# loryruta/gl-radix-sort

Measured on AMD Instinct MI355X. Metric: Mkeys/s sorting 2^28 uint32 key+val; % HBM roofline; 1/2/4/8 GPU, higher is better.
Workload: dtype u32; 1 GPU; 2^28 uint32 key + uint32 val pairs, uniform-random full-range keys, vals=iota, in-place stable radix sort, 1x MI355X; pairs_per_gpu=268435456, key_distribution=uniform, parallelism=single, device=AMD Radeon Graphics (gfx950:sramecc+:xnack-), 256 CUs, 288.0 GiB, device 0

## Files before the change

gl-radix-sort_amd/csrc/glu_sort_object.hpp:

```cpp
#pragma once
#include <algorithm>
#include <chrono>
#include <cmath>
#include <cstdlib>
#include <cstring>
#include <mutex>
#include <string>
#include <vector>

#include "glu_batch_host.hpp"
#include "radix_sort_kernels.hpp"

namespace glu_hip
{
namespace host
{
constexpr int kMaxRadix = 256;
constexpr int kMaxBlocksPerCu = 4;

template<int THREADS_, int KPT_, int BLOCKS_PER_CU_, bool CARRY_>
struct Geometry
{
    static constexpr int THREADS = THREADS_, KPT = KPT_, BLOCKS_PER_CU = BLOCKS_PER_CU_, TILE = THREADS_ * KPT_;
    static constexpr bool CARRY = CARRY_;
};
template<typename KeyT, int BITS, bool LARGE>
struct PairGeometry;
template<> struct PairGeometry<uint32_t, 8, true> : Geometry<1024, 12, 1, true> {};
template<> struct PairGeometry<uint32_t, 4, true> : Geometry<1024, 12, 1, true> {};
#ifndef GLU_SMALL_THREADS
#define GLU_SMALL_THREADS 512
#define GLU_SMALL_KPT 8
#define GLU_SMALL_BLOCKS_PER_CU 3
#endif
template<> struct PairGeometry<uint32_t, 8, false> : Geometry<GLU_SMALL_THREADS, GLU_SMALL_KPT, GLU_SMALL_BLOCKS_PER_CU, false> {};
template<> struct PairGeometry<uint32_t, 4, false> : Geometry<GLU_SMALL_THREADS, GLU_SMALL_KPT, GLU_SMALL_BLOCKS_PER_CU, false> {};
template<> struct PairGeometry<uint64_t, 8, true> : Geometry<512, 16, 1, true> {};
template<> struct PairGeometry<uint64_t, 4, true> : Geometry<1024, 8, 1, true> {};
template<> struct PairGeometry<uint64_t, 8, false> : Geometry<256, 8, 4, false> {};
template<> struct PairGeometry<uint64_t, 4, false> : Geometry<256, 8, 4, false> {};
template<typename KeyT, int BITS, bool LARGE, bool VALS = true>
struct GeometryFor : PairGeometry<KeyT, BITS, LARGE> {};
template<> struct GeometryFor<uint32_t, 8, true, false> : Geometry<1024, 20, 1, true> {};

#ifndef GLU_LINES_KPT_U32
#define GLU_LINES_KPT_U32 10
#endif
#ifndef GLU_LINES_KPT_U64
#define GLU_LINES_KPT_U64 6
#endif
template<typename KeyT, int BITS, bool VALS>
struct LinesGeometry : Geometry<1024, GLU_LINES_KPT_U32, 1, true> {};
#ifndef GLU_LINES_KPT_SEG
#define GLU_LINES_KPT_SEG 10
#endif
struct SegLinesGeometry : Geometry<1024, GLU_LINES_KPT_SEG, 1, true> {};
template<> struct LinesGeometry<uint32_t, 8, false> : Geometry<1024, 16, 1, true> {};
template<> struct LinesGeometry<uint32_t, 4, true> : Geometry<1024, 12, 1, true> {};
template<> struct LinesGeometry<uint32_t, 4, false> : Geometry<1024, 16, 1, true> {};
template<> struct LinesGeometry<uint64_t, 8, true> : Geometry<1024, GLU_LINES_KPT_U64, 1, true> {};
template<> struct LinesGeometry<uint64_t, 8, false> : Geometry<1024, 10, 1, true> {};
#ifndef GLU_LINES_KPT_U64_4BIT
#define GLU_LINES_KPT_U64_4BIT 8
#endif
template<> struct LinesGeometry<uint64_t, 4, true> : Geometry<1024, GLU_LINES_KPT_U64_4BIT, 1, true> {};
template<> struct LinesGeometry<uint64_t, 4, false> : Geometry<1024, 10, 1, true> {};
}
}

using namespace glu_hip;
using namespace glu_hip::host;

struct glu_radix_sort_s
{
    Scratch keys;
    Scratch vals;
    Scratch table;
    Scratch plan;
    Scratch pair_t2;
    Scratch pair_table;
    Scratch pair_ranges;
    Scratch pair_sub;
    Scratch pair_wide;
    Scratch seg_desc;
    Scratch seg_zero;
    bool last_planned = false;
    Scratch batch_lists;
    LastBatch last_batch;
    struct SegStage
    {
        void* host = nullptr;
        size_t size = 0;
        hipEvent_t copied = nullptr;
        bool in_flight = false;
    };
    SegStage seg_stage[16];
    uint32_t seg_stage_next = 0;
    Scratch long_image, long_hdr;
    Scratch long_bits;
    Scratch seg_gate;
    bool seg_finish = true;
    bool last_seg_finish_attempted = false;
    uint32_t last_seg_finish_capacity = 0, last_seg_finish_runs = 0, last_seg_finish_tile = 0, last_seg_finish_split = 0;
    uint32_t seg_split_max = 0;
    uint32_t seg_split_min = 0;
    uint32_t finish_rank_bits = 16;
    uint32_t seg_split_geo = 3;
    uint32_t seg_max_geo = 4;
    uint32_t digit_bits = 8;
    uint32_t max_blocks = 0;
    uint32_t reserved_cus = 0;
    bool force_small = false;
    bool no_single_block = false;
    bool no_fused_scan = false;
    bool no_plan = false;
    bool tune_scratch = true;
    bool tuning = false;
    uint32_t tuned_spacer_mib = 0, tuned_candidates = 0; double tuned_ms = 0, tuned_worst_ms = 0;
    bool no_lines = false;
    bool nt_stores = true;
    size_t nt_min_bytes = (size_t) 320 << 20;
    bool no_bit_shortcut = false;
    bool equal_shares = false;
    bool pairs = true;
    uint32_t last_pair_roles[kPlanMaxPasses] = {};
    size_t pair_min = 0;
    uint32_t pair_unit_div = 16;
    hipEvent_t after_histogram_event = nullptr;
    Scratch finish_lengths;
    Scratch finish_starts;
    Scratch finish_crowded;
    hipStream_t side = nullptr;
    hipEvent_t ev_fork = nullptr, ev_unit = nullptr, ev_fork2 = nullptr, ev_join = nullptr;
    bool fork_behind = true;
    bool ensure_side()
    {
        if (side) return true;
        if (hipStreamCreateWithFlags(&side, hipStreamNonBlocking) != hipSuccess) return side = nullptr, false;
        for (hipEvent_t* e : {&ev_fork, &ev_unit, &ev_fork2, &ev_join})
            if (hipEventCreateWithFlags(e, hipEventDisableTiming) != hipSuccess) return false;
        return true;
    }
    bool lds_finish = true;
    bool long_runs = true;
    size_t finish_min = 0;
    uint32_t* finish_hint = nullptr;
    uint32_t finish_seq = 0, finish_seq_acted_on = 0, finish_wait = 0;
    uint32_t finish_last_geo = 0;
    bool finish_last_refused = false;
    bool device_top = true;
    uint32_t top_floor = 0;
    bool last_device_top = false;
    uint32_t finish_top = 0;
    uint32_t last_finish_top = 0;
    uint32_t finish_backoff = 0;
    bool last_finish_attempted = false;
    bool last_finish_long_ok = false;
    uint32_t last_finish_capacity = 0;
    size_t large_min = 0;
    int profiling = 0;
    std::vector<hipEvent_t> events;
    size_t events_used = 0;
    std::vector<hipEvent_t> slots;
    hipEvent_t next_event()
    {
        if (events_used == events.size())
        {
            hipEvent_t e;
            if (hipEventCreate(&e) != hipSuccess) return nullptr;
            events.push_back(e);
        }
        return events[events_used++];
    }
    std::vector<uint8_t> pass_kinds;
    std::vector<uint32_t> pass_seqs;
    uint32_t cur_seq = 0;
    Scratch finish_outcomes;
    uint8_t cur_kind = 0;
    bool cur_behind = false;
    void mark(hipStream_t stream, bool around_data_kernel = false)
    {
        if (!profiling) return;
        if (slots.size() % 4 == 0) pass_kinds.push_back(cur_kind), pass_seqs.push_back(cur_seq);
        hipEvent_t e = nullptr;
        if (profiling == 1 || (around_data_kernel && !cur_behind))
            if ((e = next_event()) != nullptr) (void) hipEventRecord(e, stream);
        slots.push_back(e);
    }
};

namespace glu_hip
{
namespace host
{
constexpr size_t kPairMinKeyBytes = (size_t) 1 << 28;
constexpr size_t finish_min_count(size_t key_size) { return key_size == 8 ? (size_t) 3 << 21 : (size_t) 7 << 22; }
constexpr size_t kPlanMinCount = (size_t) 1 << 22;

inline uint32_t usable_cus(const glu_radix_sort_s* s)
{
    return (uint32_t) std::max<int>(1, g_dev.num_cus - (int) s->reserved_cus);
}

struct PlanArgs
{
    PassPlan* plan = nullptr;
    uint32_t pass = 0;
    bool may_skip = false;
    int pair_role = 0;
    uint32_t shift2 = 0, bits2 = 0;
    uint32_t flags = 0;
    bool behind_attempt = false;
    uint32_t finish_geo_first = 0, finish_geo_last = 0;
    uint32_t finish_first_ordinary = 0, finish_num_ordinary = 0;
    uint32_t finish_seq = 0, finish_top_bit = 0, finish_key_bits = 0;
    bool finish_long_ok = false;
    bool fork_side = false;
    bool unitsum_side = false;
};

constexpr size_t kSmallResidentPerCU = 4;

template<typename KeyT, int BITS>
size_t large_tiles_from(const glu_radix_sort_s* s, bool vals, size_t large_tile)
{
    if (s->large_min) return s->large_min;
    size_t from = (size_t) g_dev.num_cus * large_tile * 3 / 2;
    const size_t small_tile = vals ? GeometryFor<KeyT, BITS, false, true>::TILE : GeometryFor<KeyT, BITS, false, false>::TILE;
    if (sizeof(KeyT) == 4 && vals) from = std::max<size_t>(from, (size_t) g_dev.num_cus * kSmallResidentPerCU * small_tile + 1);
    if (sizeof(KeyT) == 4 && !vals && BITS == 8) from = std::max<size_t>(from, (size_t) 1 << 25);
    return from;
}

template<typename KeyT, int BITS>
bool lines_applicable(const glu_radix_sort_s* s, const void* src_k, const void* src_v, const void* dst_k, const void* dst_v, size_t count)
{
    const bool vals = src_v != nullptr;
    const size_t lines_tile = vals ? LinesGeometry<KeyT, BITS, true>::TILE : LinesGeometry<KeyT, BITS, false>::TILE;
    const bool aligned = (((uintptr_t) src_k | (uintptr_t) src_v | (uintptr_t) dst_k | (uintptr_t) dst_v) & 15u) == 0;
    return aligned && !s->no_lines && !s->force_small && count >= lines_tile && count >= large_tiles_from<KeyT, BITS>(s, vals, lines_tile);
}

glu_status sort_prepare_plain(glu_radix_sort_s* s, size_t count, size_t key_size, bool with_vals);
glu_status sort_typed_one_queue(glu_radix_sort_s* s, void* keys, uint32_t* vals, size_t count, glu_key_type key_type, hipStream_t stream);

template<typename KeyT>
glu_status dispatch_pass(glu_radix_sort_s* s, const KeyT* src_k, const uint32_t* src_v, KeyT* dst_k, uint32_t* dst_v,
                         size_t count, uint32_t shift, uint32_t bits, uint32_t* histogram_out, hipStream_t stream,
                         uint32_t xform = 0, PlanArgs pa = PlanArgs());
extern template glu_status dispatch_pass<uint32_t>(glu_radix_sort_s*, const uint32_t*, const uint32_t*, uint32_t*, uint32_t*, size_t, uint32_t,
                                                   uint32_t, uint32_t*, hipStream_t, uint32_t, PlanArgs);
extern template glu_status dispatch_pass<uint64_t>(glu_radix_sort_s*, const uint64_t*, const uint32_t*, uint64_t*, uint32_t*, size_t, uint32_t,
                                                   uint32_t, uint32_t*, hipStream_t, uint32_t, PlanArgs);
}
}
```

gl-radix-sort_amd/csrc/radix_pair_passes.hpp:

```cpp
#pragma once

#include "radix_sort_kernels.hpp"

namespace glu_hip
{
constexpr uint32_t kPairRadix = 256;
constexpr uint32_t kPairRowWords = kPairRadix / 2;
constexpr uint32_t kPairMaxRunUnits = 2048;

__device__ __forceinline__ uint32_t pair_word(uint32_t d, uint32_t e) { return d * kPairRowWords + ((e >> 1) ^ (d & 63u)); }

struct PairCountSmem
{
    static constexpr int WAVES = 16;
    uint32_t hist1[WAVES][kPairRadix];
    uint32_t hist2[kPairRadix * kPairRowWords];
};

constexpr uint32_t kPairWideRows = 14;
constexpr uint32_t kPairWideStride = 16 + kPairWideRows * 256;

template<typename KeyT, int TILE, bool XF = false, bool COLLECT = false>
__global__ __launch_bounds__(1024) void radix_pair_count_kernel(const KeyT* __restrict__ keys_a, uint32_t* __restrict__ table,
                                                                uint32_t* __restrict__ t2, uint32_t n, uint32_t shift,
                                                                uint32_t mask, uint32_t shift2, uint32_t mask2,
                                                                uint32_t tiles_total, uint32_t xform, const KeyT* keys_b,
                                                                PassPlan* plan, uint32_t pass, uint32_t plan_flags = 0,
                                                                uint32_t share = 0, uint32_t* __restrict__ wide = nullptr)
{
    constexpr int THREADS = 1024;
    constexpr int WAVES = PairCountSmem::WAVES;
    extern __shared__ __attribute__((aligned(16))) unsigned char smem_raw[];
    PairCountSmem& s = *reinterpret_cast<PairCountSmem*>(smem_raw);
    const uint32_t tid = threadIdx.x, lane = tid & 63, wave = tid >> 6;
    const KeyT* __restrict__ keys = keys_a;
    if (plan)
    {
        shift -= plan->shift_down[pass];
        shift2 -= plan->shift_down[pass + 1];
        if (plan->off[pass] || ((plan_flags & kPlanShortcut) && plan_digit_is_constant(plan, shift, mask)))
        {
            if (blockIdx.x == 0 && tid == 0)
            {
                plan->skip[pass] = kSkipWithoutCounting;
                plan->pair_fallback[pass + 1] = 1;
            }
            return;
        }
        if (pass > 0 && plan->flip[pass]) keys = keys_b;
        if (blockIdx.x == 0 && tid == 0)
        {
            plan->skip[pass] = 0;
            if (COLLECT && (plan_flags & kPlanCollectBits)) plan->bits_valid = 1;
        }
    }
    KeyT acc_or = 0, acc_and = (KeyT) ~(KeyT) 0;
    for (uint32_t i = tid; i < sizeof(PairCountSmem) / 4; i += THREADS) reinterpret_cast<uint32_t*>(&s)[i] = 0;
    __syncthreads();

    uint64_t begin, end;
    block_range(blockIdx.x, gridDim.x, tiles_total, TILE, n, share, begin, end);
    uint32_t* my_hist = s.hist1[wave];
    const KeyCodec<KeyT, XF> codec_in(xform & 3u);

    auto both_digits = [&](KeyT raw) {
        const KeyT k = codec_in.encode(raw);
        return digit_of<KeyT>(k, shift, mask) | (digit_of<KeyT>(k, shift2, mask2) << 8);
    };
    constexpr int VEC = 16 / sizeof(KeyT);
    using VecT = typename std::conditional<sizeof(KeyT) == 4, uint4, ulonglong2>::type;
    const bool vec_ok = (reinterpret_cast<uintptr_t>(keys) & 15u) == 0;
    const uint64_t nvec = vec_ok ? (end - begin) / VEC : 0;
    const VecT* vkeys = reinterpret_cast<const VecT*>(keys + begin);
    auto count_keys = [&](auto&& add, auto collect) {
        constexpr bool kCollect = decltype(collect)::value;
        TallyRun run;
        auto tally = [&](auto peel, KeyT raw) { wave_tally_mode(peel, both_digits(raw), lane, run, add); };
        auto tally_one = [&](KeyT raw) {
            if (kCollect) acc_or |= raw, acc_and &= raw;
            add(both_digits(raw), 1u);
        };
        auto tally_vec = [&](auto peel, const VecT& a) {
            if constexpr (sizeof(KeyT) == 4)
            {
                if (kCollect) acc_or |= a.x | a.y | a.z | a.w, acc_and &= a.x & a.y & a.z & a.w;
                tally(peel, a.x); tally(peel, a.y); tally(peel, a.z); tally(peel, a.w);
            }
            else
            {
                if (kCollect) acc_or |= a.x | a.y, acc_and &= a.x & a.y;
                tally(peel, a.x); tally(peel, a.y);
            }
        };
        uint64_t vbase = 0;
        auto main_loop = [&](auto peel) {
            for (; vbase + 4 * THREADS <= nvec; vbase += 4 * THREADS)
            {
                if (wave_tally_gives_up(peel, run)) break;
                VecT a = load_streaming(&vkeys[vbase + tid]);
                VecT b = load_streaming(&vkeys[vbase + tid + THREADS]);
                VecT c = load_streaming(&vkeys[vbase + tid + 2 * THREADS]);
                VecT d = load_streaming(&vkeys[vbase + tid + 3 * THREADS]);
                tally_vec(peel, a);
                tally_vec(peel, b);
                tally_vec(peel, c);
                tally_vec(peel, d);
            }
        };
        if (4 * THREADS <= nvec) wave_tally_dispatch(both_digits(vkeys[tid].x), lane, run, main_loop, add);
        uint64_t i = begin + vbase * VEC + tid;
        for (; i + 7ull * THREADS < end; i += 8ull * THREADS)
        {
            KeyT k[8];
#pragma unroll
            for (int j = 0; j < 8; j++) k[j] = keys[i + (uint64_t) j * THREADS];
#pragma unroll
            for (int j = 0; j < 8; j++) tally_one(k[j]);
        }
        for (; i < end; i += THREADS) tally_one(keys[i]);
    };
    auto add_count = [&](uint32_t de, uint32_t c) {
        atomicAdd(&my_hist[de & 255u], c);
        atomicAdd(&s.hist2[pair_word(de & 255u, de >> 8)], c << (16u * ((de >> 8) & 1u)));
    };
    count_keys(add_count, std::integral_constant<bool, COLLECT>());
    __syncthreads();
    if (COLLECT && (plan_flags & kPlanCollectBits)) plan_publish_bits<KeyT>(plan, acc_or, acc_and, lane);

    const uint32_t nb = gridDim.x, b = blockIdx.x;
    if (tid < kPairRadix)
    {
        uint32_t c = 0;
#pragma unroll
        for (int w = 0; w < WAVES; w++) c += s.hist1[w][tid];
        table[(size_t) tid * nb + b] = c;
        s.hist1[0][tid] = c;
    }
    __syncthreads();
    bool bad = false;
    for (uint32_t d = wave; d < kPairRadix; d += WAVES)
    {
        const uint32_t j0 = lane ^ (d & 63u);
        const uint32_t w0 = s.hist2[d * kPairRowWords + lane], w1 = s.hist2[d * kPairRowWords + 64 + lane];
        uint32_t sum = (w0 & 0xFFFFu) + (w0 >> 16) + (w1 & 0xFFFFu) + (w1 >> 16);
#pragma unroll
        for (int o = 32; o > 0; o >>= 1) sum += __shfl_xor(sum, o);
        bad = bad || sum != s.hist1[0][d];
        uint32_t* row = t2 + ((size_t) d * nb + b) * kPairRowWords;
        row[j0] = w0;
        row[64 + j0] = w1;
    }
    if (bad && lane == 0 && plan) plan->pair_fallback[pass + 1] = 1;
    if (!wide) return;
    __shared__ uint32_t nwide, wide_d[kPairWideRows];
    uint32_t* const slot_of = s.hist1[1];
    uint32_t* const wide_cnt = &s.hist1[2][0];
    static_assert(2 + kPairWideRows <= PairCountSmem::WAVES, "the wide counters live in the wave-private T1 rows, which are done with");
    __syncthreads();
    for (uint32_t i = tid; i < (1u + kPairWideRows) * kPairRadix; i += THREADS) s.hist1[1][i] = 0u;
    if (tid == 0) nwide = 0;
    __syncthreads();
    for (uint32_t d = wave; d < kPairRadix; d += WAVES)
    {
        const uint32_t w0 = s.hist2[d * kPairRowWords + lane], w1 = s.hist2[d * kPairRowWords + 64 + lane];
        uint32_t sum = (w0 & 0xFFFFu) + (w0 >> 16) + (w1 & 0xFFFFu) + (w1 >> 16);
#pragma unroll
        for (int o = 32; o > 0; o >>= 1) sum += __shfl_xor(sum, o);
        if (sum != s.hist1[0][d] && lane == 0)
        {
            const uint32_t k = atomicAdd(&nwide, 1u);
            if (k < kPairWideRows) slot_of[d] = k + 1u, wide_d[k] = d;
        }
    }
    __syncthreads();
    const uint32_t nw = nwide;
    uint32_t* const hdr = wide + (size_t) b * kPairWideStride;
    bool one_value = false;
    if (COLLECT && nw != 0)
    {
        KeyT o = acc_or, a = acc_and;
#pragma unroll
        for (int sh = 32; sh > 0; sh >>= 1)
        {
            o |= (KeyT) __shfl_xor((unsigned long long) o, sh);
            a &= (KeyT) __shfl_xor((unsigned long long) a, sh);
        }
        KeyT* const wave_bits = reinterpret_cast<KeyT*>(&s.hist2[0]);
        __syncthreads();
        if (lane == 0) wave_bits[2 * wave] = o, wave_bits[2 * wave + 1] = a;
        __syncthreads();
        o = 0, a = (KeyT) ~(KeyT) 0;
        for (int w = 0; w < WAVES; w++) o |= wave_bits[2 * w], a &= wave_bits[2 * w + 1];
        one_value = o == a;
        __syncthreads();
    }
    if (nw == 0 || nw > kPairWideRows || one_value)
    {
        if (tid == 0) hdr[0] = nw == 0 ? 0u : 0xFFFFFFFFu;
        return;
    }
    auto add_wide = [&](uint32_t de, uint32_t c) {
        const uint32_t sl = slot_of[de & 255u];
        if (sl) atomicAdd(&wide_cnt[(sl - 1u) * kPairRadix + (de >> 8)], c);
    };
    count_keys(add_wide, std::false_type());
    __syncthreads();
    if (tid == 0) hdr[0] = nw;
    if (tid < nw) hdr[1 + tid] = wide_d[tid];
    for (uint32_t k = 0; k < nw; k++)
    {
        const uint32_t d = wide_d[k];
        if (tid < kPairRadix) hdr[16 + k * kPairRadix + tid] = wide_cnt[k * kPairRadix + tid] >> 16;
        if (tid < kPairRowWords)
            t2[((size_t) d * nb + b) * kPairRowWords + tid] =
                (wide_cnt[k * kPairRadix + 2 * tid] & 0xFFFFu) | (wide_cnt[k * kPairRadix + 2 * tid + 1] << 16);
    }
}


template<int RADIX>
__device__ __forceinline__ void pair_unit_bases(const uint32_t* __restrict__ totals_l, uint32_t n, uint32_t* base, uint32_t* tmp)
{
    const uint32_t tid = threadIdx.x, lane = tid & 63, wave = tid >> 6;
    const uint32_t t = tid < (uint32_t) RADIX ? totals_l[tid] : 0u;
    uint32_t wtotal;
    uint32_t excl = wave_exclusive_sum(t, lane, wtotal);
    if (lane == 0) tmp[wave] = wtotal;
    __syncthreads();
    excl += sum_of_preceding_waves(tmp, 4, wave < 4 ? wave : 0, lane);
    if (tid < (uint32_t) RADIX) base[tid] = excl;
    if (tid == 0) base[RADIX] = n;
    __syncthreads();
}

template<int RADIX>
__device__ __forceinline__ void pair_find_run(const uint32_t* __restrict__ scanned, uint32_t row_len, const uint32_t* base,
                                              uint32_t* found, uint32_t n, uint32_t w, uint32_t nb, uint32_t (&edge)[2],
                                              uint32_t (&edge_start)[2])
{
    const uint32_t tid = threadIdx.x;
#pragma unroll
    for (int side = 0; side < 2; side++)
    {
        const uint32_t P = (uint32_t) ((uint64_t) n * (w + side) / nb);
        if (w + side == nb)
        {
            edge[side] = (uint32_t) RADIX * row_len;
            edge_start[side] = n;
            continue;
        }
        if (tid < 2) found[tid] = 0;
        __syncthreads();
        if (tid < (uint32_t) RADIX && base[tid] < P) atomicAdd(&found[0], 1u);
        __syncthreads();
        const uint32_t below = found[0];
        if (below == 0)
        {
            edge[side] = 0;
            edge_start[side] = 0;
            continue;
        }
        const uint32_t ds = below - 1;
        uint32_t mine = 0;
        for (uint32_t i = tid; i < row_len; i += blockDim.x)
            if (base[ds] + scanned[(size_t) ds * row_len + i] < P) mine++;
        if (mine) atomicAdd(&found[1], mine);
        __syncthreads();
        const uint32_t in_row = found[1];
        edge[side] = ds * row_len + in_row;
        edge_start[side] = in_row < row_len ? base[ds] + scanned[(size_t) ds * row_len + in_row] : base[ds + 1];
        __syncthreads();
    }
}

static __global__ __launch_bounds__(1024) void radix_pair_unitsum_kernel(const uint32_t* __restrict__ t2,
                                                                  const uint32_t* __restrict__ table_l,
                                                                  const uint32_t* __restrict__ totals_l,
                                                                  uint32_t* __restrict__ table_f, uint2* __restrict__ ranges,
                                                                  uint32_t n, PassPlan* plan, uint32_t pass,
                                                                  uint32_t shift = 0, uint32_t mask = 0, uint32_t plan_flags = 0)
{
    if (plan->off[pass])
    {
        if (blockIdx.x == 0 && threadIdx.x == 0) plan->skip[pass] = kSkipWithoutCounting;
        return;
    }
    if (plan->pair_fallback[pass]) return;
    shift -= plan->shift_down[pass];
    if ((plan_flags & kPlanShortcut) && plan_digit_is_constant(plan, shift, mask))
    {
        if (blockIdx.x == 0 && threadIdx.x == 0) plan->skip[pass] = kSkipWithoutCounting;
        return;
    }
    __shared__ uint32_t base[kPairRadix + 1];
    __shared__ uint32_t tmp[16];
    __shared__ uint32_t found[2];
    __shared__ uint32_t part[32][kPairRadix];
    const uint32_t tid = threadIdx.x;
    const uint32_t nb = gridDim.x, w = blockIdx.x;
    if (w == 0 && tid == 0) plan->skip[pass] = 0;
    pair_unit_bases<kPairRadix>(totals_l, n, base, tmp);
    uint32_t edge[2], edge_start[2];
    pair_find_run<kPairRadix>(table_l, nb, base, found, n, w, nb, edge, edge_start);

    if (edge[1] - edge[0] > kPairMaxRunUnits)
    {
        if (tid == 0) plan->pair_fallback[pass] = 1;
        return;
    }
    const uint32_t g = tid >> 5, q = tid & 31u;
    uint32_t acc[8] = {0, 0, 0, 0, 0, 0, 0, 0};
    const uint4* rows = reinterpret_cast<const uint4*>(t2);
#pragma unroll 4
    for (uint32_t u = edge[0] + g; u < edge[1]; u += 32)
    {
        const uint4 v = rows[(size_t) u * (kPairRowWords / 4) + q];
        acc[0] += v.x & 0xFFFFu, acc[1] += v.x >> 16, acc[2] += v.y & 0xFFFFu, acc[3] += v.y >> 16;
        acc[4] += v.z & 0xFFFFu, acc[5] += v.z >> 16, acc[6] += v.w & 0xFFFFu, acc[7] += v.w >> 16;
    }
#pragma unroll
    for (int k = 0; k < 8; k++) part[g][8 * q + k] = acc[k];
    __syncthreads();
    if (tid < kPairRadix)
    {
        uint32_t c = 0;
#pragma unroll
        for (int k = 0; k < 32; k++) c += part[k][tid];
        table_f[(size_t) tid * nb + w] = c;
    }
    if (tid == 0) ranges[w] = make_uint2(edge_start[0], edge_start[1]);
}

constexpr uint32_t kPairSub = 16;
constexpr uint32_t kPair4Radix = 16;

template<typename KeyT, int TILE, bool XF = false, bool COLLECT = false>
__global__ __launch_bounds__(256) void radix_pair4_count_kernel(const KeyT* __restrict__ keys_a, uint32_t* __restrict__ table_sub,
                                                                uint32_t* __restrict__ t2, uint32_t n, uint32_t shift,
                                                                uint32_t mask, uint32_t shift2, uint32_t mask2,
                                                                uint32_t tiles_total, uint32_t xform, const KeyT* keys_b,
                                                                PassPlan* plan, uint32_t pass, uint32_t plan_flags = 0,
                                                                uint32_t share = 0)
{
    constexpr int THREADS = 256;
    constexpr int WAVES = THREADS / kWave;
    __shared__ uint32_t hist[WAVES][256];
    const uint32_t tid = threadIdx.x, lane = tid & 63, wave = tid >> 6;
    const uint32_t nb = gridDim.x / kPairSub, b = blockIdx.x / kPairSub, j = blockIdx.x % kPairSub;
    const KeyT* __restrict__ keys = keys_a;
    if (plan)
    {
        if ((plan_flags & kPlanShortcut) && plan_digit_is_constant(plan, shift, mask))
        {
            if (blockIdx.x == 0 && tid == 0)
            {
                plan->skip[pass] = kSkipWithoutCounting;
                plan->pair_fallback[pass + 1] = 1;
            }
            return;
        }
        if (pass > 0 && plan->flip[pass]) keys = keys_b;
        if (blockIdx.x == 0 && tid == 0)
        {
            plan->skip[pass] = 0;
            if (COLLECT && (plan_flags & kPlanCollectBits)) plan->bits_valid = 1;
        }
    }
    KeyT acc_or = 0, acc_and = (KeyT) ~(KeyT) 0;
    for (int i = tid; i < WAVES * 256; i += THREADS) (&hist[0][0])[i] = 0;
    __syncthreads();
    uint64_t begin, end;
    if (share)
    {
        uint64_t b0, b1;
        block_range(b, nb, tiles_total, TILE, n, share, b0, b1);
        const uint32_t sub = ((share + kPairSub - 1) / kPairSub + 63u) & ~63u;
        begin = b0 + (uint64_t) j * sub;
        if (begin > b1) begin = b1;
        end = begin + sub;
        if (end > b1) end = b1;
    }
    else
    {
        uint32_t first, last, sf, sl;
        block_tile_range(b, nb, tiles_total, first, last);
        block_tile_range(j, kPairSub, last - first, sf, sl);
        begin = (uint64_t) (first + sf) * TILE;
        end = (uint64_t) (first + sl) * TILE;
        if (end > n) end = n;
    }
    uint32_t* my_hist = hist[wave];
    const KeyCodec<KeyT, XF> codec_in(xform & 3u);
    auto combined = [&](KeyT raw) {
        const KeyT k = codec_in.encode(raw);
        return digit_of<KeyT>(k, shift, mask) | (digit_of<KeyT>(k, shift2, mask2) << 4);
    };
    TallyRun run;
    auto add_count = [&](uint32_t cv, uint32_t c) { atomicAdd(&my_hist[cv], c); };
    auto tally = [&](auto peel, KeyT raw) { wave_tally_mode(peel, combined(raw), lane, run, add_count); };
    constexpr int VEC = 16 / sizeof(KeyT);
    using VecT = typename std::conditional<sizeof(KeyT) == 4, uint4, ulonglong2>::type;
    const bool vec_ok = (reinterpret_cast<uintptr_t>(keys) & 15u) == 0;
    auto tally_vec = [&](auto peel, const VecT& a) {
        if constexpr (sizeof(KeyT) == 4)
        {
            if (COLLECT) acc_or |= a.x | a.y | a.z | a.w, acc_and &= a.x & a.y & a.z & a.w;
            tally(peel, a.x); tally(peel, a.y); tally(peel, a.z); tally(peel, a.w);
        }
        else
        {
            if (COLLECT) acc_or |= a.x | a.y, acc_and &= a.x & a.y;
            tally(peel, a.x); tally(peel, a.y);
        }
    };
    if (begin < end)
    {
        const uint64_t nvec = vec_ok ? (end - begin) / VEC : 0;
        const VecT* vkeys = reinterpret_cast<const VecT*>(keys + begin);
        uint64_t vbase = 0;
        auto main_loop = [&](auto peel) {
            for (; vbase + 4 * THREADS <= nvec; vbase += 4 * THREADS)
            {
                if (wave_tally_gives_up(peel, run)) break;
                VecT a = load_streaming(&vkeys[vbase + tid]);
                VecT bq = load_streaming(&vkeys[vbase + tid + THREADS]);
                VecT c = load_streaming(&vkeys[vbase + tid + 2 * THREADS]);
                VecT d = load_streaming(&vkeys[vbase + tid + 3 * THREADS]);
                tally_vec(peel, a);
                tally_vec(peel, bq);
                tally_vec(peel, c);
                tally_vec(peel, d);
            }
        };
        if (4 * THREADS <= nvec) wave_tally_dispatch(combined(vkeys[tid].x), lane, run, main_loop, add_count);
        for (uint64_t i = begin + vbase * VEC + tid; i < end; i += THREADS)
        {
            const KeyT raw = keys[i];
            if (COLLECT) acc_or |= raw, acc_and &= raw;
            atomicAdd(&my_hist[combined(raw)], 1u);
        }
    }
    __syncthreads();
    if (COLLECT && (plan_flags & kPlanCollectBits)) plan_publish_bits<KeyT>(plan, acc_or, acc_and, lane);
    uint32_t c = 0;
#pragma unroll
    for (int wv = 0; wv < WAVES; wv++) c += hist[wv][tid];
    t2[(size_t) blockIdx.x * 256 + (tid & 15u) * 16 + (tid >> 4)] = c;
    uint32_t sum = c;
    sum += __shfl_xor(sum, 16);
    sum += __shfl_xor(sum, 32);
    __syncthreads();
    if (lane < 16) hist[wave][lane] = sum;
    __syncthreads();
    if (tid < kPair4Radix)
        table_sub[(size_t) tid * gridDim.x + blockIdx.x] = hist[0][tid] + hist[1][tid] + hist[2][tid] + hist[3][tid];
}

static __global__ __launch_bounds__(1024) void radix_pair4_unitsum_kernel(const uint32_t* __restrict__ t2,
                                                                   const uint32_t* __restrict__ sub_scanned,
                                                                   const uint32_t* __restrict__ totals_l,
                                                                   uint32_t* __restrict__ table_f, uint2* __restrict__ ranges,
                                                                   uint32_t n, PassPlan* plan, uint32_t pass,
                                                                   uint32_t shift = 0, uint32_t mask = 0, uint32_t plan_flags = 0)
{
    if (plan->pair_fallback[pass]) return;
    if ((plan_flags & kPlanShortcut) && plan_digit_is_constant(plan, shift, mask))
    {
        if (blockIdx.x == 0 && threadIdx.x == 0) plan->skip[pass] = kSkipWithoutCounting;
        return;
    }
    __shared__ uint32_t base[kPair4Radix + 1];
    __shared__ uint32_t tmp[16];
    __shared__ uint32_t found[2];
    __shared__ uint32_t part[64][kPair4Radix];
    const uint32_t tid = threadIdx.x;
    const uint32_t nb = gridDim.x, w = blockIdx.x;
    const uint32_t row_len = nb * kPairSub;
    if (w == 0 && tid == 0) plan->skip[pass] = 0;
    pair_unit_bases<kPair4Radix>(totals_l, n, base, tmp);
    uint32_t edge[2], edge_start[2];
    pair_find_run<kPair4Radix>(sub_scanned, row_len, base, found, n, w, nb, edge, edge_start);
    if (edge[1] - edge[0] > kPairMaxRunUnits * 4)
    {
        if (tid == 0) plan->pair_fallback[pass] = 1;
        return;
    }
    const uint32_t g = tid >> 4, e = tid & 15u;
    uint32_t acc = 0;
#pragma unroll 4
    for (uint32_t u = edge[0] + g; u < edge[1]; u += 64)
    {
        const uint32_t d = u / row_len, i = u % row_len;
        acc += t2[(size_t) i * 256 + d * 16 + e];
    }
    part[g][e] = acc;
    __syncthreads();
    if (tid < kPair4Radix)
    {
        uint32_t c = 0;
#pragma unroll
        for (int k = 0; k < 64; k++) c += part[k][tid];
        table_f[(size_t) tid * nb + w] = c;
    }
    if (tid == 0) ranges[w] = make_uint2(edge_start[0], edge_start[1]);
}

}
```

Baseline: 74890 Mkeys/s.

## Drop per-wave first-digit histograms; derive counts from packed pair rows with overflow recount

```diff
diff --git a/gl-radix-sort_amd/csrc/glu_sort_object.hpp b/gl-radix-sort_amd/csrc/glu_sort_object.hpp
--- a/gl-radix-sort_amd/csrc/glu_sort_object.hpp
+++ b/gl-radix-sort_amd/csrc/glu_sort_object.hpp
@@ -136,9 +136,18 @@
     bool ensure_side()
     {
         if (side) return true;
-        if (hipStreamCreateWithFlags(&side, hipStreamNonBlocking) != hipSuccess) return side = nullptr, false;
+        hipStream_t st = nullptr;
+        if (hipStreamCreateWithFlags(&st, hipStreamNonBlocking) != hipSuccess) return (void) hipGetLastError(), false;
         for (hipEvent_t* e : {&ev_fork, &ev_unit, &ev_fork2, &ev_join})
-            if (hipEventCreateWithFlags(e, hipEventDisableTiming) != hipSuccess) return false;
+            if (hipEventCreateWithFlags(e, hipEventDisableTiming) != hipSuccess)
+            {
+                (void) hipGetLastError();
+                for (hipEvent_t* made : {&ev_fork, &ev_unit, &ev_fork2, &ev_join})
+                    if (*made) (void) hipEventDestroy(*made), *made = nullptr;
+                (void) hipStreamDestroy(st);
+                return false;
+            }
+        side = st;
         return true;
     }
     bool lds_finish = true;
diff --git a/gl-radix-sort_amd/csrc/radix_pair_passes.hpp b/gl-radix-sort_amd/csrc/radix_pair_passes.hpp
--- a/gl-radix-sort_amd/csrc/radix_pair_passes.hpp
+++ b/gl-radix-sort_amd/csrc/radix_pair_passes.hpp
@@ -13,8 +13,9 @@
 struct PairCountSmem
 {
     static constexpr int WAVES = 16;
-    uint32_t hist1[WAVES][kPairRadix];
     uint32_t hist2[kPairRadix * kPairRowWords];
+    uint32_t row_sum[kPairRadix];
+    unsigned long long wave_bits[2 * WAVES];
 };
 
 constexpr uint32_t kPairWideRows = 14;
@@ -60,7 +61,6 @@
 
     uint64_t begin, end;
     block_range(blockIdx.x, gridDim.x, tiles_total, TILE, n, share, begin, end);
-    uint32_t* my_hist = s.hist1[wave];
     const KeyCodec<KeyT, XF> codec_in(xform & 3u);
 
     auto both_digits = [&](KeyT raw) {
@@ -119,25 +119,13 @@
         }
         for (; i < end; i += THREADS) tally_one(keys[i]);
     };
-    auto add_count = [&](uint32_t de, uint32_t c) {
-        atomicAdd(&my_hist[de & 255u], c);
+    const uint32_t nb = gridDim.x, b = blockIdx.x;
+    auto add_pair = [&](uint32_t de, uint32_t c) {
         atomicAdd(&s.hist2[pair_word(de & 255u, de >> 8)], c << (16u * ((de >> 8) & 1u)));
     };
-    count_keys(add_count, std::integral_constant<bool, COLLECT>());
+    count_keys(add_pair, std::integral_constant<bool, COLLECT>());
     __syncthreads();
     if (COLLECT && (plan_flags & kPlanCollectBits)) plan_publish_bits<KeyT>(plan, acc_or, acc_and, lane);
-
-    const uint32_t nb = gridDim.x, b = blockIdx.x;
-    if (tid < kPairRadix)
-    {
-        uint32_t c = 0;
-#pragma unroll
-        for (int w = 0; w < WAVES; w++) c += s.hist1[w][tid];
-        table[(size_t) tid * nb + b] = c;
-        s.hist1[0][tid] = c;
-    }
-    __syncthreads();
-    bool bad = false;
     for (uint32_t d = wave; d < kPairRadix; d += WAVES)
     {
         const uint32_t j0 = lane ^ (d & 63u);
@@ -145,38 +133,28 @@
         uint32_t sum = (w0 & 0xFFFFu) + (w0 >> 16) + (w1 & 0xFFFFu) + (w1 >> 16);
 #pragma unroll
         for (int o = 32; o > 0; o >>= 1) sum += __shfl_xor(sum, o);
-        bad = bad || sum != s.hist1[0][d];
+        if (lane == 0) s.row_sum[d] = sum;
         uint32_t* row = t2 + ((size_t) d * nb + b) * kPairRowWords;
         row[j0] = w0;
         row[64 + j0] = w1;
     }
-    if (bad && lane == 0 && plan) plan->pair_fallback[pass + 1] = 1;
-    if (!wide) return;
+    __syncthreads();
+    uint32_t* const hdr = wide ? wide + (size_t) b * kPairWideStride : nullptr;
+    {
+        uint32_t total = s.row_sum[lane] + s.row_sum[64 + lane] + s.row_sum[128 + lane] + s.row_sum[192 + lane];
+#pragma unroll
+        for (int o = 32; o > 0; o >>= 1) total += __shfl_xor(total, o);
+        if (total == (uint32_t) (end - begin))
+        {
+            if (tid < kPairRadix) table[(size_t) tid * nb + b] = s.row_sum[tid];
+            if (hdr && tid == 0) hdr[0] = 0u;
+            return;
+        }
+    }
     __shared__ uint32_t nwide, wide_d[kPairWideRows];
-    uint32_t* const slot_of = s.hist1[1];
-    uint32_t* const wide_cnt = &s.hist1[2][0];
-    static_assert(2 + kPairWideRows <= PairCountSmem::WAVES, "the wide counters live in the wave-private T1 rows, which are done with");
-    __syncthreads();
-    for (uint32_t i = tid; i < (1u + kPairWideRows) * kPairRadix; i += THREADS) s.hist1[1][i] = 0u;
-    if (tid == 0) nwide = 0;
-    __syncthreads();
-    for (uint32_t d = wave; d < kPairRadix; d += WAVES)
-    {
-        const uint32_t w0 = s.hist2[d * kPairRowWords + lane], w1 = s.hist2[d * kPairRowWords + 64 + lane];
-        uint32_t sum = (w0 & 0xFFFFu) + (w0 >> 16) + (w1 & 0xFFFFu) + (w1 >> 16);
-#pragma unroll
-        for (int o = 32; o > 0; o >>= 1) sum += __shfl_xor(sum, o);
-        if (sum != s.hist1[0][d] && lane == 0)
-        {
-            const uint32_t k = atomicAdd(&nwide, 1u);
-            if (k < kPairWideRows) slot_of[d] = k + 1u, wide_d[k] = d;
-        }
-    }
-    __syncthreads();
-    const uint32_t nw = nwide;
-    uint32_t* const hdr = wide + (size_t) b * kPairWideStride;
     bool one_value = false;
-    if (COLLECT && nw != 0)
+    KeyT the_value = 0;
+    if (COLLECT)
     {
         KeyT o = acc_or, a = acc_and;
 #pragma unroll
@@ -185,35 +163,66 @@
             o |= (KeyT) __shfl_xor((unsigned long long) o, sh);
             a &= (KeyT) __shfl_xor((unsigned long long) a, sh);
         }
-        KeyT* const wave_bits = reinterpret_cast<KeyT*>(&s.hist2[0]);
-        __syncthreads();
-        if (lane == 0) wave_bits[2 * wave] = o, wave_bits[2 * wave + 1] = a;
+        if (lane == 0) s.wave_bits[2 * wave] = o, s.wave_bits[2 * wave + 1] = a;
         __syncthreads();
         o = 0, a = (KeyT) ~(KeyT) 0;
-        for (int w = 0; w < WAVES; w++) o |= wave_bits[2 * w], a &= wave_bits[2 * w + 1];
+        for (int w = 0; w < WAVES; w++) o |= (KeyT) s.wave_bits[2 * w], a &= (KeyT) s.wave_bits[2 * w + 1];
         one_value = o == a;
-        __syncthreads();
-    }
+        the_value = o;
+    }
+    for (uint32_t i = tid; i < kPairRadix * kPairRowWords; i += THREADS) s.hist2[i] = 0;
+    if (tid == 0) nwide = 0;
+    __syncthreads();
+    if (one_value)
+    {
+        const uint32_t de = both_digits(the_value);
+        if (tid == 0) s.hist2[pair_word(de & 255u, de >> 8)] = (uint32_t) (end - begin);
+    }
+    else
+    {
+        auto add_sum = [&](uint32_t de, uint32_t c) { atomicAdd(&s.hist2[pair_word(de & 255u, de >> 8)], c); };
+        count_keys(add_sum, std::false_type());
+    }
+    __syncthreads();
+    for (uint32_t d = wave; d < kPairRadix; d += WAVES)
+    {
+        uint32_t sum = s.hist2[d * kPairRowWords + lane] + s.hist2[d * kPairRowWords + 64 + lane];
+#pragma unroll
+        for (int o = 32; o > 0; o >>= 1) sum += __shfl_xor(sum, o);
+        if (lane == 0)
+        {
+            table[(size_t) d * nb + b] = sum;
+            if (sum != s.row_sum[d])
+            {
+                const uint32_t k = atomicAdd(&nwide, 1u);
+                if (k < kPairWideRows) wide_d[k] = d;
+            }
+        }
+    }
+    __syncthreads();
+    const uint32_t nw = nwide;
+    if (nw != 0 && tid == 0 && plan) plan->pair_fallback[pass + 1] = 1;
+    if (!hdr) return;
     if (nw == 0 || nw > kPairWideRows || one_value)
     {
         if (tid == 0) hdr[0] = nw == 0 ? 0u : 0xFFFFFFFFu;
         return;
     }
-    auto add_wide = [&](uint32_t de, uint32_t c) {
-        const uint32_t sl = slot_of[de & 255u];
-        if (sl) atomicAdd(&wide_cnt[(sl - 1u) * kPairRadix + (de >> 8)], c);
-    };
-    count_keys(add_wide, std::false_type());
-    __syncthreads();
     if (tid == 0) hdr[0] = nw;
     if (tid < nw) hdr[1 + tid] = wide_d[tid];
     for (uint32_t k = 0; k < nw; k++)
     {
         const uint32_t d = wide_d[k];
-        if (tid < kPairRadix) hdr[16 + k * kPairRadix + tid] = wide_cnt[k * kPairRadix + tid] >> 16;
         if (tid < kPairRowWords)
-            t2[((size_t) d * nb + b) * kPairRowWords + tid] =
-                (wide_cnt[k * kPairRadix + 2 * tid] & 0xFFFFu) | (wide_cnt[k * kPairRadix + 2 * tid + 1] << 16);
+        {
+            uint32_t* const word = t2 + ((size_t) d * nb + b) * kPairRowWords + tid;
+            const uint32_t w = __hip_atomic_load(word, __ATOMIC_RELAXED, __HIP_MEMORY_SCOPE_WORKGROUP), lo = w & 0xFFFFu, hi = w >> 16;
+            const uint32_t p = s.hist2[d * kPairRowWords + (tid ^ (d & 63u))];
+            const uint32_t even = lo + (((hi + lo - p) & 0xFFFFu) << 16), odd = p - even;
+            hdr[16 + k * kPairRadix + 2 * tid] = even >> 16;
+            hdr[16 + k * kPairRadix + 2 * tid + 1] = odd >> 16;
+            *word = lo | (odd << 16);
+        }
     }
 }
 
```

After: 74010 Mkeys/s. 0.988x the previous value.
